# JiaweiXu8/AD-GS

Measured on AMD Instinct MI355X. Metric: fwd+bwd frames/s, higher is better.
Workload: dtype f32; 1 GPU; C3: 1000000 Gaussians, 1920x1280, SH deg 3, 8 dynamic objects, flow+semantic outputs, 1 camera/GPU/step; P=1000000, camera_pool=16 cameras / time stamps per GPU, cycled one per step (train.py:55-61), settle_steps=123, capacity_reruns=0, launch=eager, parallelism=single GPU, gradient_exchange=none, camera_streams=1

## Files before the change

ad-gs_amd/adgs/_lib.py:

```python
import contextlib
import ctypes
import os

_HERE = os.path.dirname(os.path.abspath(__file__))
PKG_ROOT = os.path.dirname(_HERE)
LIB_PATH = os.environ.get("ADGS_LIB") or os.path.join(PKG_ROOT, "lib", "libadgs_hip.so")

ALLOC_FN = ctypes.CFUNCTYPE(ctypes.c_void_p, ctypes.c_void_p, ctypes.c_size_t)

_lib = None

c_p = ctypes.c_void_p
c_i = ctypes.c_int
c_f = ctypes.c_float

SIGNATURES = {
    "adgs_last_error": (ctypes.c_char_p, []),
    "adgs_device_check": (c_i, []),
    "adgs_raster_forward": (c_i, [ALLOC_FN, c_p, ALLOC_FN, c_p, ALLOC_FN, c_p, c_i, c_i, c_i, c_i, c_p, c_i, c_i,
                                  c_p, c_p, c_p, c_p, c_p, c_p, c_p, c_f, c_p, c_p, c_p, c_p, c_p, c_f, c_f, c_i,
                                  c_p, c_p, c_p, c_p, c_p, c_i, c_p, c_i, c_p]),
    "adgs_raster_render": (c_i, [ALLOC_FN, c_p, ALLOC_FN, c_p, ALLOC_FN, c_p, c_i, c_i, c_i, c_i, c_p, c_i, c_i,
                                 c_p, c_p, c_p, c_p, c_p, c_p, c_p, c_f, c_p, c_p, c_p, c_p, c_p, c_f, c_f, c_i,
                                 c_p, c_p, c_p, c_p, c_p, c_i, c_p, c_i, c_p]),
# ... 128 lines not shown
    "adgs_mesh_normals_temp_bytes": (ctypes.c_size_t, [ctypes.c_longlong, ctypes.c_longlong]),
    "adgs_mesh_vertex_normals": (c_i, [c_i, c_i, c_p, c_p, c_p, c_p, c_p]),
    "adgs_geometry_grid_temp_bytes": (ctypes.c_size_t, [ctypes.c_longlong]),
    "adgs_geometry_grid_plan": (c_i, [c_i, c_p, c_f, c_p, c_p, c_p, c_p, c_p]),
    "adgs_geometry_grid_build": (c_i, [c_i, c_p, c_f, c_p, c_p, c_p, c_p, c_p, c_p, c_p, c_p]),
    "adgs_geometry_nearest_temp_bytes": (ctypes.c_size_t, [ctypes.c_longlong]),
    "adgs_geometry_nearest": (c_i, [c_i, c_i, c_p, c_f, c_f, c_p, c_p, c_p, c_p, c_p, c_p, c_p, c_p, c_p, c_p]),
    "adgs_geometry_face_areas": (c_i, [c_i, c_i, c_p, c_p, c_p, c_p]),
    "adgs_geometry_sample": (c_i, [c_i, c_i, c_i, c_p, c_p, c_p, ctypes.c_double, ctypes.c_ulonglong, c_p, c_p, c_p]),
    "adgs_geometry_stats_temp_bytes": (ctypes.c_size_t, [ctypes.c_longlong]),
    "adgs_geometry_distance_stats": (c_i, [c_i, c_p, c_i, c_p, ctypes.c_double, c_p, c_p, c_p]),
    "adgs_simplify_cluster_temp_bytes": (ctypes.c_size_t, [ctypes.c_longlong, ctypes.c_longlong]),
    "adgs_simplify_cluster": (c_i, [c_i, c_i, c_p, c_p, c_f, c_p, c_p, c_p, c_p, c_p]),
    "adgs_simplify_cluster_emit": (c_i, [c_i, c_i, c_p, c_p, c_p, c_p, c_p, c_p, c_p, c_p, c_p, c_p, c_p]),
    "adgs_simplify_place_temp_bytes": (ctypes.c_size_t, [ctypes.c_longlong, ctypes.c_longlong]),
    "adgs_simplify_place": (c_i, [c_i, c_i, c_i, c_i, c_p, c_p, c_p, c_p, c_p, c_p, c_f, c_p, c_i, ctypes.c_double, c_p, c_p, c_p, c_p]),
    "adgs_test_v2_published_entries": (ctypes.c_longlong, [c_p, c_i, c_i, c_p]),
    "adgs_test_v2_scanned_candidates": (ctypes.c_longlong, [c_p, c_i, c_i, c_p]),
    "adgs_test_v2_tile_counters": (ctypes.c_longlong, [c_p, c_i, c_i, c_p, c_p, ctypes.c_longlong, c_p]),
    "adgs_test_v2_blend_batches": (ctypes.c_longlong, [c_p, c_i, c_i, c_p]),
    "adgs_test_v2_cell_ranges": (ctypes.c_longlong, [c_p, c_i, c_i, c_p, ctypes.c_longlong, c_p]),
    "adgs_test_v2_published_mask": (ctypes.c_longlong, [c_p, c_i, c_p, c_p, c_p]),
    "adgs_test_v2_geom_offsets": (c_i, [c_i, c_p]),
    "adgs_test_abi_sizeof": (ctypes.c_size_t, [c_i]),
    "adgs_test_set_capacity_hints": (None, [ctypes.c_longlong, ctypes.c_longlong]),
    "adgs_test_env_reads": (ctypes.c_ulonglong, []),
    "adgs_test_scramble_slab_bounds": (c_i, [ctypes.c_uint]),
    "adgs_test_scan_temp_bytes": (ctypes.c_size_t, [ctypes.c_size_t]),
    "adgs_test_exclusive_scan_u32": (c_i, [c_p, c_p, ctypes.c_size_t, c_p, c_p]),
    "adgs_test_sort_temp_bytes": (ctypes.c_size_t, [ctypes.c_size_t]),
    "adgs_test_sort_pairs_u64": (c_i, [c_p, c_p, c_p, c_p, ctypes.c_size_t, c_i, c_p, c_p]),
    "adgs_test_sort_pairs_u32": (c_i, [c_p, c_p, c_p, c_p, ctypes.c_size_t, c_i, c_p, c_p]),
    "adgs_test_bilagrid_path": (c_i, [c_i, c_i, c_i, c_i, c_i]),
    "adgs_test_deform_plan": (c_i, [c_p, c_i, c_i, c_i, c_p, c_p, c_p, c_p, c_p, c_p, c_p, c_p, c_p, c_p]),
}


class RasterOptions(ctypes.Structure):
    _fields_ = [("struct_bytes", ctypes.c_uint64), ("antialiasing", ctypes.c_int32)]


def raster_options(antialiasing=False):
    o = RasterOptions()
    o.struct_bytes = ctypes.sizeof(RasterOptions)
    o.antialiasing = 1 if antialiasing else 0
    return o
# ... 106 lines not shown
```

ad-gs_amd/csrc/api.hip:

```cpp
#include "common.h"
#include "kernels.h"
#include "../../include/adgs_rasterizer.h"
#include "../../include/adgs_optim.h"

#include <atomic>
#include <chrono>
#include <mutex>
#include <vector>
#include <cstdlib>
#include <algorithm>
#include <cmath>
#include <cstring>

namespace adgs {

static thread_local std::string g_last_error;
struct FrameContext {
	adgs_frame_stats stats;
	size_t hint_cells, hint_fine;
	unsigned hint_max_cell_chunks;
	bool bucket_frame_pending;
	long long reruns;
	int last_order_hint;
	uint32_t* slab_bounds;
// ... 236 lines not shown
			if (captured) return nullptr;
			for (Entry& c : entries) if (!c.captured && (!e || c.used < e->used)) e = &c;
			if (!e) return nullptr;
			(void)hipStreamSynchronize(e->stream);
			if (e->tiles != tiles || e->extra != extra) { (void)hipFree(e->buf); e->buf = nullptr; e->tiles = 0; e->view = nullptr; if (hipMalloc((void**)&e->buf, (tiles + 16 + extra) * sizeof(uint32_t)) != hipSuccess) { e->buf = nullptr; return nullptr; } }
		} else {
			Entry fresh{ nullptr, nullptr, 0, 0, 0, nullptr, false, nullptr, 0, false, 0 };
			if (hipMalloc((void**)&fresh.buf, (tiles + 16 + extra) * sizeof(uint32_t)) != hipSuccess) return nullptr;
			entries.push_back(fresh);
			e = &entries.back();
		}
		e->view = view; e->proj = proj; e->W = W; e->H = H; e->tiles = tiles; e->stream = stream; e->captured = captured; e->used = ++clock; e->written = false; e->extra = extra;
		if (!reset_signature(e->buf, tiles, extra)) { e->view = nullptr; e->tiles = 0; (void)hipFree(e->buf); e->buf = nullptr; return nullptr; }
		return e;
	}
};
static OrderHints* order_hints() {
	constexpr int MAX_DEV = 64;
	static thread_local OrderHints hints[MAX_DEV];
	int dev = 0;
	if (hipGetDevice(&dev) != hipSuccess || dev < 0 || dev >= MAX_DEV) return nullptr;
	return &hints[dev];
}
struct FrameCfg { int v2; int cell_tiles; int ppl; int tile_order = 1; int sh_staging = 1; int timeline = 0; int order_ready = 0; int backwards = 0; int antialiasing = 0; int published = 0; int prefill = 0; };
static uint32_t frame_cfg_word(const FrameCfg& c) {
	return 0xAD600000u | ((uint32_t)(c.v2 & 1) << 19) | ((uint32_t)(c.tile_order & 1) << 18) | ((uint32_t)(c.sh_staging & 1) << 17) | ((uint32_t)(c.timeline & 1) << 16) |
	       ((uint32_t)(c.order_ready & 1) << 15) | ((uint32_t)(c.antialiasing & 1) << 14) | ((uint32_t)(c.published & 1) << 13) |
	       ((uint32_t)(c.prefill & 1) << 12) | ((uint32_t)(c.ppl & 0x7) << 8) | (uint32_t)(c.cell_tiles & 0xff);
}
static bool frame_cfg_from_word(uint32_t w, FrameCfg* c) {
	if ((w & 0xFFF00000u) != 0xAD600000u) return false;
	*c = FrameCfg{ (int)((w >> 19) & 1u), (int)(w & 0xffu), (int)((w >> 8) & 0x7u) };
	c->tile_order = (int)((w >> 18) & 1u); c->sh_staging = (int)((w >> 17) & 1u); c->timeline = (int)((w >> 16) & 1u); c->order_ready = (int)((w >> 15) & 1u);
	c->antialiasing = (int)((w >> 14) & 1u); c->published = (int)((w >> 13) & 1u); c->prefill = (int)((w >> 12) & 1u) & c->published;
	return c->cell_tiles >= 1 && (c->ppl == 1 || c->ppl == 2 || c->ppl == 4);
}
struct FrameKey {
	const void* img; const void* geom; int W, H, P;
	bool operator==(const FrameKey& o) const { return img == o.img && geom == o.geom && W == o.W && H == o.H && P == o.P; }
};
static std::mutex g_cfg_mu;
static std::vector<std::pair<FrameKey, FrameCfg>> g_cfg_table;
static void remember_frame(const FrameKey& k, const FrameCfg& c) {
	std::lock_guard<std::mutex> lk(g_cfg_mu);
	for (auto it = g_cfg_table.begin(); it != g_cfg_table.end();) it = (it->first.img == k.img || it->first.geom == k.geom) ? g_cfg_table.erase(it) : it + 1;
	if (g_cfg_table.size() >= 256) g_cfg_table.erase(g_cfg_table.begin());
	g_cfg_table.emplace_back(k, c);
}
static int note_backward(const FrameKey& k) {
	std::lock_guard<std::mutex> lk(g_cfg_mu);
	for (auto it = g_cfg_table.rbegin(); it != g_cfg_table.rend(); ++it) if (it->first == k) return it->second.backwards++;
	return -1;
}
static bool lookup_frame(const FrameKey& k, FrameCfg* c) {
	std::lock_guard<std::mutex> lk(g_cfg_mu);
	for (auto it = g_cfg_table.rbegin(); it != g_cfg_table.rend(); ++it) if (it->first == k) { *c = it->second; return true; }
	return false;
// ... 145 lines not shown
		size_t gb = 0, ib = 0;
		const size_t count_cells = buckets ? ncells : 0;
		const bool with_ddir = training && sh_src && M == 16;
		GeomStateV2::carve(nullptr, P, &gb, with_ddir, count_cells);
		char* gch = geometryBuffer(geometryUser, gb);
		const int ppl = v2_pixels_per_lane(ntiles), sub = TILE_Y / (4 * ppl);
		const int wgy = (height + 4 * ppl - 1) / (4 * ppl);
		const size_t wtiles = (size_t)gx * wgy;
		ImgStateV2::carve(nullptr, npix, wtiles, ncells, &ib);
		char* ich = imageBuffer(imageUser, ib);
		if (!gch || !ich) { set_error("buffer allocator returned NULL"); return -1; }
		GeomStateV2 geom = GeomStateV2::carve(gch, P, nullptr, with_ddir, count_cells);
		ImgStateV2 img = ImgStateV2::carve(ich, npix, wtiles, ncells, nullptr);
		uint32_t frame_word = 0; bool order_tiles = false;
		{
			FrameCfg fcfg{ 1, cell_tiles, ppl };
			fcfg.antialiasing = antialiasing ? 1 : 0;
			fcfg.tile_order = env_int("ADGS_TILE_ORDER", 1) != 0; fcfg.sh_staging = env_str("ADGS_NO_SH_STAGING") == nullptr; fcfg.timeline = env_int("ADGS_TIMELINE_BWD", 0) != 0;
			order_tiles = wtiles >= 2048 && fcfg.tile_order;
			if (!training) order_tiles = false;
			fcfg.order_ready = order_tiles ? 1 : 0;
			fcfg.published = (training && env_int("ADGS_PUBLISHED_MASK", 1) != 0) ? 1 : 0;
			fcfg.prefill = (fcfg.published && env_int("ADGS_GRAD_PREFILL", 1) != 0) ? 1 : 0;
			if (training) remember_frame(FrameKey{ ich, gch, width, height, P }, fcfg);
			frame_word = frame_cfg_word(fcfg);
		}
		const int fwd_order_mode = env_int("ADGS_FWD_ORDER", 2);
		OrderHints::Entry* hint = nullptr;
		const uint32_t* hint_read = nullptr;
		const bool fwd_hint_wanted = wtiles >= 2048 && env_int("ADGS_TILE_ORDER", 1) != 0 && fwd_order_mode == 2;
		if (fwd_hint_wanted) {
			hipStreamCaptureStatus cs0 = hipStreamCaptureStatusNone;
			(void)hipStreamIsCapturing(stream, &cs0);
			if (OrderHints* oh = order_hints()) {
				const bool cap0 = cs0 == hipStreamCaptureStatusActive;
				hint = oh->find(viewmatrix, projmatrix, width, height, wtiles, stream, cap0);
				if (!hint && training) {
					hipStreamCaptureMode mode = hipStreamCaptureModeRelaxed;
					if (cap0) (void)hipThreadExchangeStreamCaptureMode(&mode);
					hint = oh->create(viewmatrix, projmatrix, width, height, wtiles, stream, cap0, std::min<size_t>(ncells, (size_t)MAX_CELLS) * SLAB_ROW);
					if (cap0) (void)hipThreadExchangeStreamCaptureMode(&mode);
					(void)hipGetLastError();
				}
				oh->lookups++;
				if (hint && hint->buf) { hint_read = hint->buf; if (hint->written) oh->hits++; fc->last_order_hint = hint->written ? 1 : 0; } else { hint = nullptr; fc->last_order_hint = 0; }
			}
// ... 354 lines not shown
		ra.tile_order = nullptr;
		ra.tl_start = cfg.timeline ? img.tile_scanned : nullptr; ra.tl_end = img.tile_batches;
		PreprocessBwdArgs pa;
		pa.P = P; pa.D = D; pa.M = M;
		pa.means3D = means3D; pa.radii = radii; pa.shs = shs; pa.clamped = geom.clamped;
		pa.scales = scales; pa.rotations = rotations; pa.scale_modifier = scale_modifier;
		pa.cov3D = cov3D_precomp;
		pa.view = viewmatrix; pa.proj = projmatrix; pa.campos = campos;
		pa.focal_y = height / (2.0f * tan_fovy); pa.focal_x = width / (2.0f * tan_fovx);
		pa.tan_fovx = tan_fovx; pa.tan_fovy = tan_fovy; pa.inv_depth = inv_depth;
		pa.dL_dmean2D = nullptr; pa.dL_dconic = nullptr; pa.dL_dcolor = nullptr; pa.dL_ddepth = nullptr;
		pa.dL_dmean3D = dL_dmean3D; pa.dL_dcov3D = dL_dcov3D; pa.dL_dsh = dL_dsh; pa.dL_dscale = dL_dscale; pa.dL_drot = dL_drot;
		pa.gacc = geom.gacc; pa.splats = geom.splats; pa.W = width; pa.H = height;
		memset(&pa.sh_src, 0, sizeof(pa.sh_src)); pa.sh_dst = ShGradDst{};
		if (sh_src) { pa.sh_src = *sh_src; if (sh_dst) pa.sh_dst = *sh_dst; }
		pa.out_mean2D = dL_dmean2D; pa.out_conic = dL_dconic; pa.out_opacity = dL_dopacity; pa.out_color = dL_dcolor; pa.out_depth = dL_ddepth;
		pa.out_flow = ra.do_flow ? dL_dflow : nullptr; pa.out_sem = ra.do_sem ? dL_dsemantic : nullptr; pa.D_S = D_S;
		pa.out_mean2D_abs = dL_dmean2D_abs;
		pa.sh_staging = cfg.sh_staging;
		pa.ddir = geom.ddir;
		pa.antialias = cfg.antialiasing;
		pa.published = cfg.published ? geom.published : nullptr;
		pa.prefill = (cfg.prefill && cfg.published) ? 1 : 0;
		const FillPlan fill = preprocess_bwd_fill_plan(pa);
		{
			StageTimer t(ST_RENDER_BWD, stream);
			if (wtiles >= 2048 && cfg.tile_order) {
				if (!cfg.order_ready && launch_tile_order((int)wtiles, img.tile_consumed, img.tile_order, stream) != 0) return -1;
				ra.tile_order = img.tile_order;
			}
			if (note_backward(fkey) != 0) ADGS_HIP_CHECK(hipMemsetAsync(geom.gacc, 0, (size_t)P * GACC_STRIDE * sizeof(float), stream));
			ra.sem_src = nullptr; ra.sem_dst = nullptr; ra.sem_stride = 0;
			if (binning_buffer && launch_render_bwd_v2(ra, stream, pa.prefill ? &fill : nullptr) != 0) return -1;
			if (!binning_buffer && pa.prefill && launch_grad_prefill(fill, stream) != 0) return -1;
			if (binning_buffer && ra.do_sem && D_S > 1) {
				ADGS_HIP_CHECK(hipMemsetAsync(dL_dsemantic, 0, (size_t)P * D_S * sizeof(float), stream));
				RenderV2BwdArgs rc = ra;
				rc.do_color = rc.do_flow = rc.do_depth = rc.do_opacity = false; rc.do_sem = true; rc.absgrad = false;
				rc.dL_dpix = nullptr; rc.dL_dpix_depth = nullptr; rc.dL_dpix_flow = nullptr; rc.dL_dpix_opacity = nullptr;
				rc.bg_image = nullptr; rc.dL_dbg_image = nullptr; rc.sem_stride = D_S;
				for (int c = 1; c < D_S; c++) {
					rc.dL_dpix_sem = dL_dpix_semantic + (size_t)c * npix; rc.sem_src = semantic + c; rc.sem_dst = dL_dsemantic + c;
					if (launch_render_bwd_v2(rc, stream) != 0) return -1;
				}
			}
		}
// ... 20 lines not shown
	ra.do_depth = dL_dpix_depth != nullptr;
	ra.do_opacity = grad_img_opacity != nullptr;
	ra.dL_dmean2D = dL_dmean2D; ra.dL_dconic = dL_dconic; ra.dL_dopacity = dL_dopacity; ra.dL_dcolor = dL_dcolor;
	ra.dL_ddepth = dL_ddepth; ra.dL_dflow = dL_dflow; ra.dL_dsem = dL_dsemantic;
	if (R > 0) {
		{ StageTimer t(ST_RENDER_BWD, stream); if (launch_render_bwd(ra, stream) != 0) return -1; }
		ADGS_LAUNCH_CHECK(debug, stream);
	}

	PreprocessBwdArgs pa;
	pa.P = P; pa.D = D; pa.M = M;
	pa.means3D = means3D; pa.radii = radii; pa.shs = shs; pa.clamped = geom.clamped;
	pa.scales = scales; pa.rotations = rotations; pa.scale_modifier = scale_modifier;
	pa.cov3D = cov3D_precomp ? cov3D_precomp : geom.cov3D;
	pa.view = viewmatrix; pa.proj = projmatrix; pa.campos = campos;
	pa.focal_y = height / (2.0f * tan_fovy); pa.focal_x = width / (2.0f * tan_fovx);
	pa.tan_fovx = tan_fovx; pa.tan_fovy = tan_fovy; pa.inv_depth = inv_depth;
	pa.dL_dmean2D = dL_dmean2D; pa.dL_dconic = dL_dconic; pa.dL_dcolor = dL_dcolor; pa.dL_ddepth = dL_ddepth;
	pa.dL_dmean3D = dL_dmean3D; pa.dL_dcov3D = dL_dcov3D; pa.dL_dsh = dL_dsh; pa.dL_dscale = dL_dscale; pa.dL_drot = dL_drot;
	if (sh_src) { set_error("the raw-SH entry points need the default (v2) pipeline (not ADGS_RASTER_MODE=classic, D_S <= ADGS_V2_MAX_SEMANTIC)"); return -1; }
	memset(&pa.sh_src, 0, sizeof(pa.sh_src)); pa.sh_dst = ShGradDst{};
	pa.gacc = nullptr; pa.splats = nullptr; pa.W = width; pa.H = height; pa.out_mean2D = nullptr; pa.out_conic = nullptr; pa.out_opacity = nullptr; pa.out_color = nullptr; pa.out_depth = nullptr;
	pa.out_flow = nullptr; pa.out_sem = nullptr; pa.D_S = D_S; pa.out_mean2D_abs = nullptr;
	pa.sh_staging = cfg.sh_staging; pa.ddir = nullptr; pa.published = nullptr; pa.prefill = 0;
	pa.antialias = cfg.antialiasing;
	if (cfg.antialiasing) { pa.out_opacity = dL_dopacity; pa.splats = geom.splats; }
	{ StageTimer t(ST_PREPROCESS_BWD, stream); if (launch_preprocess_bwd(pa, stream) != 0) return -1; }
	ADGS_LAUNCH_CHECK(debug, stream);
	return 0;
}

static int read_raster_options(const adgs_raster_options* o, const char* who, int* antialiasing) {
	*antialiasing = 0;
	if (!o) return 0;
	if (o->struct_bytes < offsetof(adgs_raster_options, antialiasing) + sizeof(int32_t) || o->struct_bytes > 4096) {
		set_error(std::string(who) + ": adgs_raster_options.struct_bytes must be sizeof(adgs_raster_options) of the caller's header"); return -1;
	}
	adgs_raster_options full;
	memset(&full, 0, sizeof(full));
	memcpy(&full, o, std::min<size_t>((size_t)o->struct_bytes, sizeof(full)));
	if (full.antialiasing != 0 && full.antialiasing != 1) { set_error(std::string(who) + ": adgs_raster_options.antialiasing must be 0 or 1"); return -1; }
	*antialiasing = full.antialiasing;
	return 0;
}

extern "C" int adgs_raster_forward_opts(
	adgs_alloc_fn geometryBuffer, void* geometryUser, adgs_alloc_fn binningBuffer, void* binningUser, adgs_alloc_fn imageBuffer, void* imageUser,
// ... 296 lines not shown
}
long long sum_tile_words(const uint32_t* d_words, size_t n, hipStream_t stream) {
	std::vector<uint32_t> h(n);
	if (hipMemcpyAsync(h.data(), d_words, n * sizeof(uint32_t), hipMemcpyDeviceToHost, stream) != hipSuccess) return -1;
	if (hipStreamSynchronize(stream) != hipSuccess) return -1;
	long long total = 0;
	for (uint32_t x : h) total += x;
	return total;
}
}
extern "C" long long adgs_test_v2_published_entries(const char* img_buffer, int width, int height, void* stream_) {
	V2ImageView v;
	if (!v2_image_view(img_buffer, width, height, &v)) return -1;
	return sum_tile_words(v.img.tile_consumed, v.wtiles, (hipStream_t)stream_);
}
extern "C" long long adgs_test_v2_published_mask(const char* geom_buffer, int P, uint8_t* out_bytes, float* out_lines, void* stream_) {
	if (!geom_buffer || P <= 0) return -1;
	const GeomStateV2 g = GeomStateV2::carve(const_cast<char*>(geom_buffer), (size_t)P, nullptr, false);
	if (out_bytes && hipMemcpyAsync(out_bytes, g.published, (size_t)P, hipMemcpyDeviceToHost, (hipStream_t)stream_) != hipSuccess) return -1;
	if (out_lines && hipMemcpyAsync(out_lines, g.gacc, (size_t)P * GACC_STRIDE * sizeof(float), hipMemcpyDeviceToHost, (hipStream_t)stream_) != hipSuccess) return -1;
	if (hipStreamSynchronize((hipStream_t)stream_) != hipSuccess) return -1;
	return (long long)P;
}
extern "C" int adgs_test_v2_geom_offsets(int P, long long* out2) {
	if (P <= 0 || !out2) return -1;
	char* const base = reinterpret_cast<char*>((uintptr_t)1 << 20);
	const GeomStateV2 g = GeomStateV2::carve(base, (size_t)P, nullptr, false);
	out2[0] = (long long)(reinterpret_cast<char*>(g.published) - base); out2[1] = (long long)(reinterpret_cast<char*>(g.gacc) - base);
	return 0;
}
extern "C" long long adgs_test_v2_tile_counters(const char* img_buffer, int width, int height, uint32_t* out_consumed, uint32_t* out_scanned, long long capacity, void* stream_) {
	V2ImageView v;
	if (!v2_image_view(img_buffer, width, height, &v)) return -1;
	if ((long long)v.wtiles > capacity) return (long long)v.wtiles;
	if (out_consumed && hipMemcpyAsync(out_consumed, v.img.tile_consumed, v.wtiles * sizeof(uint32_t), hipMemcpyDeviceToHost, (hipStream_t)stream_) != hipSuccess) return -1;
	if (out_scanned && hipMemcpyAsync(out_scanned, v.img.tile_scanned, v.wtiles * sizeof(uint32_t), hipMemcpyDeviceToHost, (hipStream_t)stream_) != hipSuccess) return -1;
	if (hipStreamSynchronize((hipStream_t)stream_) != hipSuccess) return -1;
	return (long long)v.wtiles;
}
extern "C" long long adgs_test_v2_tile_words(const char* img_buffer, int width, int height, uint32_t* out_scanned, uint32_t* out_batches, long long capacity, void* stream_) {
	V2ImageView v;
	if (!v2_image_view(img_buffer, width, height, &v)) return -1;
	if ((long long)v.wtiles > capacity) return (long long)v.wtiles;
	if (out_scanned && hipMemcpyAsync(out_scanned, v.img.tile_scanned, v.wtiles * sizeof(uint32_t), hipMemcpyDeviceToHost, (hipStream_t)stream_) != hipSuccess) return -1;
	if (out_batches && hipMemcpyAsync(out_batches, v.img.tile_batches, v.wtiles * sizeof(uint32_t), hipMemcpyDeviceToHost, (hipStream_t)stream_) != hipSuccess) return -1;
	if (hipStreamSynchronize((hipStream_t)stream_) != hipSuccess) return -1;
// ... 67 lines not shown
```

ad-gs_amd/csrc/kernels.h:

```cpp
#pragma once
#include "common.h"
#include "func_eval.h"
#include "grad_prefill.h"

namespace adgs {

struct PreprocessArgs {
	int P, D, M, D_S;
	const float* means3D; const float* scales; float scale_modifier; const float* rotations;
	const float* opacities; const float* shs; const float* cov3D_precomp; const float* colors_precomp;
	const float* flow_points; const float* semantic;
	const float* view; const float* proj; const float* campos;
	int W, H, gx, gy;
	float tan_fovx, tan_fovy, focal_x, focal_y;
	int inv_depth;
	int* radii; Splat* splats; float* cov3D; uint8_t* clamped; uint32_t* tiles_touched;
	int v2;
	uint32_t* fine_touched;
	uint4* dupinfo;
	int cell_tiles, cgx, cgy;
	ShSource sh_src;
	const float* sh0;
	float* gacc;
	unsigned long long* fine_total;
// ... 40 lines not shown
};
int launch_render_bwd(const RenderBwdArgs& a, hipStream_t stream);

struct PreprocessBwdArgs {
	int P, D, M;
	const float* means3D; const int* radii; const float* shs; const uint8_t* clamped;
	const float* scales; const float* rotations; float scale_modifier;
	const float* cov3D;
	const float* view; const float* proj; const float* campos;
	float focal_x, focal_y, tan_fovx, tan_fovy;
	int inv_depth;
	const float* dL_dmean2D; const float* dL_dconic; const float* dL_dcolor; const float* dL_ddepth;
	float* dL_dmean3D; float* dL_dcov3D; float* dL_dsh; float* dL_dscale; float* dL_drot;
	float* gacc; const Splat* splats; int W, H;
	ShSource sh_src; ShGradDst sh_dst;
	float* out_mean2D; float* out_conic; float* out_opacity; float* out_color; float* out_depth; float* out_flow; float* out_sem;
	float* out_mean2D_abs;
	int D_S;
	int sh_staging;
	const float* ddir;
	int antialias;
	const uint8_t* published;
	int prefill;
};
int launch_preprocess_bwd(const PreprocessBwdArgs& a, hipStream_t stream);
FillPlan preprocess_bwd_fill_plan(const PreprocessBwdArgs& a);

constexpr int CHUNK_WORDS = 2 + WAVE;
constexpr int CHUNK_PREV = WAVE, CHUNK_COUNT = WAVE + 1;
constexpr int POOL_BLOCK = 4;
constexpr int GACC_STRIDE = 16;
constexpr int GACC_USED = 14;

constexpr int MAX_CELLS = 1024;
constexpr int SLAB_ROW = 128;
constexpr int MAX_SLAB_LG = 7;
constexpr int SLAB_TARGET = 3072;
constexpr int SLAB_TARGET_FOREIGN = 2048;
constexpr int GS_NMAX = 4096;
constexpr int MAX_CHUNKS = 16384;
constexpr size_t count_row_stride(int nblocks) { return ((size_t)nblocks + 3u) & ~(size_t)3u; }
struct Mailbox { volatile uint32_t seq; uint32_t r_cells; unsigned long long r_fine; uint32_t oversize, n_groups, overflow, overflow_count, max_cell_chunks;
	uint32_t cap_cells; unsigned long long cap_fine; };
int launch_bin_prepare(const FramePrologue& p, hipStream_t stream);
struct CellScanArgs {
	const uint32_t* cell_count;
	uint32_t* cell_start;
	uint2* cell_ranges; int ncells;
// ... 104 lines not shown
```

ad-gs_amd/csrc/preprocess_bwd.hip:

```cpp
#include "common.h"
#include "kernels.h"
#include "geom.h"
#include "func_eval.h"
#include <cstdlib>

#ifndef ADGS_PREB_STAGE_U4
#define ADGS_PREB_STAGE_U4 12
#endif
namespace adgs {
namespace {

struct M3 { float v[3][3]; };
__device__ __forceinline__ M3 m3mul(const M3& a, const M3& b) {
	M3 r;
#pragma unroll
	for (int c = 0; c < 3; c++)
#pragma unroll
		for (int rr = 0; rr < 3; rr++)
			r.v[c][rr] = a.v[0][rr] * b.v[c][0] + a.v[1][rr] * b.v[c][1] + a.v[2][rr] * b.v[c][2];
	return r;
}
__device__ __forceinline__ M3 m3t(const M3& a) {
	M3 r;
#pragma unroll
	for (int c = 0; c < 3; c++)
#pragma unroll
// ... 11 lines not shown
	const bool rs = a.sh_src.scene_xyz != nullptr && (int)i < a.sh_src.Ns;
	in.radius = gate ? 0 : a.radii[i];
	if (!pub) return in;
	const float* pos = rs ? a.sh_src.scene_xyz : a.means3D;
	in.p[0] = pos[3 * i]; in.p[1] = pos[3 * i + 1]; in.p[2] = pos[3 * i + 2];
	const float* sc = rs ? a.sh_src.scene_scaling : a.scales;
	const float* rt = rs ? a.sh_src.scene_rotation : a.rotations;
	in.s[0] = sc[3 * i]; in.s[1] = sc[3 * i + 1]; in.s[2] = sc[3 * i + 2];
	const float4 r = *reinterpret_cast<const float4*>(rt + 4 * i);
	in.q[0] = r.x; in.q[1] = r.y; in.q[2] = r.z; in.q[3] = r.w;
	in.op = rs ? a.sh_src.scene_opacity[i] : 0.f;
	const float4* ga = reinterpret_cast<const float4*>(a.gacc + i * GACC_STRIDE);
	in.u0 = ld_stream4(ga); in.u1 = ld_stream4(ga + 1); in.u2 = ld_stream4(ga + 2); in.u3 = ld_stream4(ga + 3);
	const float4* sp = reinterpret_cast<const float4*>(a.splats + i);
	in.s0 = ld_stream4(sp); in.s1 = ld_stream4(sp + 1);
	in.clamped = a.clamped[i];
	if (a.ddir) {
#pragma unroll
		for (int k = 0; k < 9; k++) in.dd[k] = ld_stream(a.ddir + (size_t)k * a.P + i);
	}
	return in;
}

template <bool STAGED, bool AA>
__global__ void __launch_bounds__(BW_THREADS) preprocess_bwd_kernel(PreprocessBwdArgs a) {
	extern __shared__ float s_sh[];
	const int tid = threadIdx.x;
	const int base = blockIdx.x * BW_THREADS;
	const int idx = base + tid;
	const bool raw = a.sh_src.scene_dc != nullptr;
	const int nvalid = min(BW_THREADS, a.P - base);
	const bool pf = STAGED && a.gacc != nullptr && a.cov3D == nullptr && a.scales != nullptr && a.rotations != nullptr;
	const bool adam_rest = STAGED && raw && (a.sh_dst.adam.scene_rest.p != nullptr || a.sh_dst.adam.obj_rest.p != nullptr);
	const bool gate = a.gacc != nullptr && a.published != nullptr;
	bool pub = true;
	if (gate) pub = idx < a.P && a.published[idx] != 0;
	bool sparse = false;
	if (gate && a.prefill) {
		const int npub = __syncthreads_count(pub);
		sparse = prefill_group_sparse(npub, nvalid);
		if (sparse && npub == 0 && !adam_rest) return;
	}
	PreBIn in;
	const bool have_ddir = STAGED && raw && pf && a.ddir != nullptr && a.D == 3;
	if (STAGED) {
		if (raw && have_ddir) {
			in = load_preb_in(a, idx, gate, pub);
		} else if (raw) {
			stage_rows<true, ADGS_PREB_STAGE_U4>(s_sh, SH_ROW_REST, SH_ROW_REST, base, nvalid, a.sh_src.Ns, a.sh_src.scene_rest, a.sh_src.obj_rest, tid, BW_THREADS,
				[&]() { if (pf) in = load_preb_in(a, idx, gate, pub); });
		} else {
			const float4* src = reinterpret_cast<const float4*>(a.shs + (size_t)base * SH_ROW_FULL);
			constexpr int NQ4 = SH_ROW_FULL / 4;
			const int total4 = nvalid * NQ4;
			float4 v[NQ4];
#pragma unroll
			for (int u = 0; u < NQ4; u++) v[u] = ld_stream4(src + min(tid + u * BW_THREADS, total4 - 1));
			if (pf) in = load_preb_in(a, idx, gate, pub);
#pragma unroll
			for (int u = 0; u < NQ4; u++) {
				const int q = tid + u * BW_THREADS;
				if (q < total4) {
					const int g = q / NQ4, c = (q - g * NQ4) * 4;
					float* d = s_sh + g * SH_ROW_FULL_LDS + c;
					d[0] = v[u].x; d[1] = v[u].y; d[2] = v[u].z; d[3] = v[u].w;
				}
			}
// ... 308 lines not shown
		for (int k = 0; k < 3; k++) { dMt.v[0][k] *= s0; dMt.v[1][k] *= s1; dMt.v[2][k] *= s2; }
#define MT(i, j) dMt.v[i][j]
		float4 dq;
		dq.x = 2 * z * (MT(0, 1) - MT(1, 0)) + 2 * y * (MT(2, 0) - MT(0, 2)) + 2 * x * (MT(1, 2) - MT(2, 1));
		dq.y = 2 * y * (MT(1, 0) + MT(0, 1)) + 2 * z * (MT(2, 0) + MT(0, 2)) + 2 * r * (MT(1, 2) - MT(2, 1)) - 4 * x * (MT(2, 2) + MT(1, 1));
		dq.z = 2 * x * (MT(1, 0) + MT(0, 1)) + 2 * r * (MT(2, 0) - MT(0, 2)) + 2 * z * (MT(1, 2) + MT(2, 1)) - 4 * y * (MT(2, 2) + MT(0, 0));
		dq.w = 2 * r * (MT(0, 1) - MT(1, 0)) + 2 * x * (MT(2, 0) + MT(0, 2)) + 2 * y * (MT(1, 2) + MT(2, 1)) - 4 * z * (MT(1, 1) + MT(0, 0));
#undef MT
		if (rs) {
			const float qg = r * dq.x + x * dq.y + y * dq.z + z * dq.w;
			st_stream4(reinterpret_cast<float4*>(a.sh_dst.scene_rotation + 4 * (size_t)idx),
				make_float4((dq.x - r * qg) * act.inv_norm, (dq.y - x * qg) * act.inv_norm, (dq.z - y * qg) * act.inv_norm, (dq.w - z * qg) * act.inv_norm));
		} else st_stream4(reinterpret_cast<float4*>(a.dL_drot + 4 * (size_t)idx), dq);
	}
	}
	if (STAGED) {
		__syncthreads();
		if (raw && adam_rest) {
			adam_rows<4>(s_sh, SH_ROW_REST, SH_ROW_REST, base, nvalid, a.sh_src.Ns, a.sh_dst.adam.scene_rest, a.sh_dst.adam.obj_rest, a.sh_dst.adam.beta1, a.sh_dst.adam.beta2, a.sh_dst.adam.eps,
				tid, BW_THREADS);
		} else if (sparse) {
			const int lane = tid & (WAVE - 1), w0 = tid - lane;
			for (uint64_t m = __builtin_amdgcn_ballot_w64(vis); m != 0ull; m &= m - 1ull) {
				const int r = w0 + __builtin_ctzll(m), gi = base + r;
				if (raw) {
					const bool is_obj = gi >= a.sh_src.Ns;
					float* const gre = is_obj ? a.sh_dst.obj_rest : a.sh_dst.scene_rest;
					if (gre && lane < SH_ROW_REST) st_stream(gre + (size_t)(is_obj ? gi - a.sh_src.Ns : gi) * SH_ROW_REST + lane, s_sh[r * SH_ROW_REST + lane]);
				} else if (lane < SH_ROW_FULL) {
					st_stream(a.dL_dsh + (size_t)gi * SH_ROW_FULL + lane, s_sh[r * SH_ROW_FULL_LDS + lane]);
				}
			}
		} else if (raw) {
			stage_rows<false>(s_sh, SH_ROW_REST, SH_ROW_REST, base, nvalid, a.sh_src.Ns, a.sh_dst.scene_rest, a.sh_dst.obj_rest, tid, BW_THREADS);
		} else {
			float4* dst = reinterpret_cast<float4*>(a.dL_dsh + (size_t)base * SH_ROW_FULL);
			for (int q = tid; q < nvalid * (SH_ROW_FULL / 4); q += BW_THREADS) {
				const int g = q / (SH_ROW_FULL / 4), c = (q - g * (SH_ROW_FULL / 4)) * 4;
				const float* s = s_sh + g * SH_ROW_FULL_LDS + c;
				st_stream4(dst + q, make_float4(s[0], s[1], s[2], s[3]));
			}
		}
	}
}

}

// ... 17 lines not shown
		fill_plan_add(fp, a.sh_dst.scene_xyz, 3, 3, 0, Nr); fill_plan_add(fp, a.sh_dst.scene_scaling, 3, 3, 0, Nr);
		fill_plan_add(fp, a.sh_dst.scene_rotation, 4, 4, 0, Nr); fill_plan_add(fp, a.sh_dst.scene_opacity, 1, 1, 0, Nr);
	}
	tail(a.dL_dmean3D, 3);
	all(a.dL_dcov3D, 6);
	if (raw) {
		fill_plan_add(fp, a.sh_dst.scene_dc, 3, 3, 0, Ns); fill_plan_add(fp, a.sh_dst.obj_dc, 3, 3, Ns, P - Ns);
		all(a.sh_dst.rgb_factor, 3);
		const bool adam_rest = a.sh_dst.adam.scene_rest.p || a.sh_dst.adam.obj_rest.p;
		const int rest = (a.M - 1) * 3;
		if (!adam_rest) { fill_plan_add(fp, a.sh_dst.scene_rest, rest, rest, 0, Ns); fill_plan_add(fp, a.sh_dst.obj_rest, rest, rest, Ns, P - Ns); }
		const bool adam_sp = a.sh_dst.adam.scene_sp.p || a.sh_dst.adam.obj_sp.p;
		if (has_lin_host(a.sh_src.f) && !adam_sp) {
			const int row = 3 * a.sh_src.f.n_params;
			fill_plan_add(fp, a.sh_dst.scene_sp, row, row, 0, Ns); fill_plan_add(fp, a.sh_dst.obj_sp, row, row, Ns, P - Ns);
		}
	} else if (a.shs) {
		all(a.dL_dsh, a.M * 3);
	}
	if (a.scales) { tail(a.dL_dscale, 3); tail(a.dL_drot, 4); }
	return fp;
}

int launch_preprocess_bwd(const PreprocessBwdArgs& a, hipStream_t stream) {
	if (a.P == 0) return 0;
	const bool raw = a.sh_src.scene_dc != nullptr;
	const bool staged = a.M == 16 && (raw || a.shs) && a.gacc != nullptr && a.sh_staging != 0;
	const unsigned grid = (unsigned)((a.P + BW_THREADS - 1) / BW_THREADS);
	const bool adam_rest = a.sh_dst.adam.scene_rest.p || a.sh_dst.adam.obj_rest.p, adam_sp = a.sh_dst.adam.scene_sp.p || a.sh_dst.adam.obj_sp.p;
	if ((adam_rest || adam_sp) && !raw) { set_error("preprocess backward: the in-backward Adam step needs the raw-SH path"); return -1; }
	if (adam_rest && !staged) {
		set_error("preprocess backward: the in-backward Adam step of the SH `rest` tensors needs 16 SH coefficients and the LDS row staging "
		          "(the frame's forward ran with ADGS_NO_SH_STAGING, or M != 16)");
		return -1;
	}
	if (a.out_mean2D_abs && !a.gacc) { set_error("preprocess backward: the absolute mean2D gradient needs the default (v2) pipeline's accumulator lines"); return -1; }
	if (a.antialias && (!a.out_opacity || (!a.gacc && !a.splats))) { set_error("preprocess backward: the anti-aliased frame's opacity gradient has no destination"); return -1; }
	if (staged) {
		const size_t lds = (size_t)BW_THREADS * (raw ? SH_ROW_REST : SH_ROW_FULL_LDS) * sizeof(float);
		if (a.antialias) hipLaunchKernelGGL((preprocess_bwd_kernel<true, true>), dim3(grid), dim3(BW_THREADS), lds, stream, a);
		else hipLaunchKernelGGL((preprocess_bwd_kernel<true, false>), dim3(grid), dim3(BW_THREADS), lds, stream, a);
	} else {
		if (a.antialias) hipLaunchKernelGGL((preprocess_bwd_kernel<false, true>), dim3(grid), dim3(BW_THREADS), 0, stream, a);
		else hipLaunchKernelGGL((preprocess_bwd_kernel<false, false>), dim3(grid), dim3(BW_THREADS), 0, stream, a);
	}
	ADGS_HIP_CHECK(hipGetLastError());
	if (raw && has_lin_host(a.sh_src.f)) {
		const int No = a.P - a.sh_src.Ns;
		if (a.prefill && a.gacc && a.published && !adam_sp)
			return launch_lin_param_grad_rows(a.sh_src.Ns, a.sh_dst.scene_dc, a.sh_dst.scene_sp, No, a.sh_dst.obj_dc, a.sh_dst.obj_sp, 3, 3, a.sh_src.f, a.published, stream);
		if (launch_lin_param_grad2(a.sh_src.Ns, a.sh_dst.scene_dc, a.sh_dst.scene_sp, No, a.sh_dst.obj_dc, a.sh_dst.obj_sp, 3, 3, a.sh_src.f, stream,
		                           &a.sh_dst.adam.scene_sp, &a.sh_dst.adam.obj_sp, a.sh_dst.adam.beta1, a.sh_dst.adam.beta2, a.sh_dst.adam.eps) != 0) return -1;
	}
	return 0;
}

}
```

include/adgs_testing.h:

```cpp
#ifndef ADGS_TESTING_H
#define ADGS_TESTING_H
#include <stddef.h>
#include <stdint.h>
#include "adgs_deform.h"
#ifdef __cplusplus
extern "C" {
#endif
size_t adgs_test_scan_temp_bytes(size_t n);
int adgs_test_exclusive_scan_u32(const uint32_t* in, uint32_t* out, size_t n, char* temp, void* stream);
size_t adgs_test_sort_temp_bytes(size_t n);
int adgs_test_sort_pairs_u64(uint64_t* keys_in, uint64_t* keys_out, uint32_t* vals_in, uint32_t* vals_out, size_t n, int end_bit, char* temp, void* stream);
int adgs_test_sort_pairs_u32(uint32_t* keys_in, uint32_t* keys_out, uint32_t* vals_in, uint32_t* vals_out, size_t n, int end_bit, char* temp, void* stream);
long long adgs_test_v2_published_entries(const char* img_buffer, int width, int height, void* stream);
long long adgs_test_v2_scanned_candidates(const char* img_buffer, int width, int height, void* stream);
long long adgs_test_v2_tile_counters(const char* img_buffer, int width, int height, uint32_t* out_consumed, uint32_t* out_scanned, long long capacity, void* stream);
long long adgs_test_v2_blend_batches(const char* img_buffer, int width, int height, void* stream);
long long adgs_test_v2_cell_ranges(const char* img_buffer, int width, int height, uint32_t* out_ranges, long long capacity, void* stream);
long long adgs_test_v2_published_mask(const char* geom_buffer, int P, uint8_t* out_bytes, float* out_lines, void* stream);
int adgs_test_v2_geom_offsets(int P, long long* out2);

size_t adgs_test_abi_sizeof(int which);

unsigned long long adgs_test_env_reads(void);

void adgs_test_set_capacity_hints(long long pairs, long long fine_pairs);

int adgs_test_scramble_slab_bounds(unsigned seed);

int adgs_test_bilagrid_path(int L, int Hg, int Wg, int H, int W);

#define ADGS_TEST_DEFORM_PLAN_FIELDS 11
int adgs_test_deform_plan(const adgs_deform_params* p, int np_xyz, int np_xyz_flow, int np_rotation, const adgs_deform_outputs* out, const float* flow_xyz,
	const float* dL_dxyz, const float* dL_drotation, const float* dL_dopacity, const float* dL_dscales, const float* dL_dflow_xyz,
	const adgs_deform_grads* grads, int32_t* fwd, int32_t* bwd);

#ifdef __cplusplus
}
#endif
#endif
```

Before: 1128 frames/s.

## Compact sparse published Gaussians into dense span blocks in preprocess backward

Adds span blocks to the staged preprocess-backward kernel. Each span block scans BWD_SPAN groups of published-mask bytes, builds an LDS list of the published indices in sparse groups, and processes them densely. The regular per-group blocks then exit early when their group is sparse. The aim is fewer partly idle wavefronts and wasted per-block work when only a few Gaussians per group are visible. In exchange it adds extra blocks, a block-level scan with syncthreads, and scattered gathers of Gaussian data. It is on by default through ADGS_BWD_COMPACT, with a test hook to read back the span-block count.

```diff
diff --git a/ad-gs_amd/adgs/_lib.py b/ad-gs_amd/adgs/_lib.py
--- a/ad-gs_amd/adgs/_lib.py
+++ b/ad-gs_amd/adgs/_lib.py
@@ -174,6 +174,7 @@
     "adgs_test_v2_cell_ranges": (ctypes.c_longlong, [c_p, c_i, c_i, c_p, ctypes.c_longlong, c_p]),
     "adgs_test_v2_published_mask": (ctypes.c_longlong, [c_p, c_i, c_p, c_p, c_p]),
     "adgs_test_v2_geom_offsets": (c_i, [c_i, c_p]),
+    "adgs_test_preprocess_bwd_span_blocks": (c_i, []),
     "adgs_test_abi_sizeof": (ctypes.c_size_t, [c_i]),
     "adgs_test_set_capacity_hints": (None, [ctypes.c_longlong, ctypes.c_longlong]),
     "adgs_test_env_reads": (ctypes.c_ulonglong, []),
diff --git a/ad-gs_amd/csrc/api.hip b/ad-gs_amd/csrc/api.hip
--- a/ad-gs_amd/csrc/api.hip
+++ b/ad-gs_amd/csrc/api.hip
@@ -282,17 +282,18 @@
 	if (hipGetDevice(&dev) != hipSuccess || dev < 0 || dev >= MAX_DEV) return nullptr;
 	return &hints[dev];
 }
-struct FrameCfg { int v2; int cell_tiles; int ppl; int tile_order = 1; int sh_staging = 1; int timeline = 0; int order_ready = 0; int backwards = 0; int antialiasing = 0; int published = 0; int prefill = 0; };
+struct FrameCfg { int v2; int cell_tiles; int ppl; int tile_order = 1; int sh_staging = 1; int timeline = 0; int order_ready = 0; int backwards = 0; int antialiasing = 0; int published = 0; int prefill = 0; int compact = 0; };
 static uint32_t frame_cfg_word(const FrameCfg& c) {
 	return 0xAD600000u | ((uint32_t)(c.v2 & 1) << 19) | ((uint32_t)(c.tile_order & 1) << 18) | ((uint32_t)(c.sh_staging & 1) << 17) | ((uint32_t)(c.timeline & 1) << 16) |
 	       ((uint32_t)(c.order_ready & 1) << 15) | ((uint32_t)(c.antialiasing & 1) << 14) | ((uint32_t)(c.published & 1) << 13) |
-	       ((uint32_t)(c.prefill & 1) << 12) | ((uint32_t)(c.ppl & 0x7) << 8) | (uint32_t)(c.cell_tiles & 0xff);
+	       ((uint32_t)(c.prefill & 1) << 12) | ((uint32_t)(c.compact & 1) << 11) | ((uint32_t)(c.ppl & 0x7) << 8) | (uint32_t)(c.cell_tiles & 0xff);
 }
 static bool frame_cfg_from_word(uint32_t w, FrameCfg* c) {
 	if ((w & 0xFFF00000u) != 0xAD600000u) return false;
 	*c = FrameCfg{ (int)((w >> 19) & 1u), (int)(w & 0xffu), (int)((w >> 8) & 0x7u) };
 	c->tile_order = (int)((w >> 18) & 1u); c->sh_staging = (int)((w >> 17) & 1u); c->timeline = (int)((w >> 16) & 1u); c->order_ready = (int)((w >> 15) & 1u);
 	c->antialiasing = (int)((w >> 14) & 1u); c->published = (int)((w >> 13) & 1u); c->prefill = (int)((w >> 12) & 1u) & c->published;
+	c->compact = (int)((w >> 11) & 1u) & c->prefill;
 	return c->cell_tiles >= 1 && (c->ppl == 1 || c->ppl == 2 || c->ppl == 4);
 }
 struct FrameKey {
@@ -484,6 +485,7 @@
 			fcfg.order_ready = order_tiles ? 1 : 0;
 			fcfg.published = (training && env_int("ADGS_PUBLISHED_MASK", 1) != 0) ? 1 : 0;
 			fcfg.prefill = (fcfg.published && env_int("ADGS_GRAD_PREFILL", 1) != 0) ? 1 : 0;
+			fcfg.compact = (fcfg.prefill && env_int("ADGS_BWD_COMPACT", 1) != 0) ? 1 : 0;
 			if (training) remember_frame(FrameKey{ ich, gch, width, height, P }, fcfg);
 			frame_word = frame_cfg_word(fcfg);
 		}
@@ -884,6 +886,7 @@
 		pa.antialias = cfg.antialiasing;
 		pa.published = cfg.published ? geom.published : nullptr;
 		pa.prefill = (cfg.prefill && cfg.published) ? 1 : 0;
+		pa.compact = (cfg.compact && pa.prefill) ? 1 : 0; pa.span_blocks = 0;
 		const FillPlan fill = preprocess_bwd_fill_plan(pa);
 		{
 			StageTimer t(ST_RENDER_BWD, stream);
@@ -950,7 +953,7 @@
 	memset(&pa.sh_src, 0, sizeof(pa.sh_src)); pa.sh_dst = ShGradDst{};
 	pa.gacc = nullptr; pa.splats = nullptr; pa.W = width; pa.H = height; pa.out_mean2D = nullptr; pa.out_conic = nullptr; pa.out_opacity = nullptr; pa.out_color = nullptr; pa.out_depth = nullptr;
 	pa.out_flow = nullptr; pa.out_sem = nullptr; pa.D_S = D_S; pa.out_mean2D_abs = nullptr;
-	pa.sh_staging = cfg.sh_staging; pa.ddir = nullptr; pa.published = nullptr; pa.prefill = 0;
+	pa.sh_staging = cfg.sh_staging; pa.ddir = nullptr; pa.published = nullptr; pa.prefill = 0; pa.compact = 0; pa.span_blocks = 0;
 	pa.antialias = cfg.antialiasing;
 	if (cfg.antialiasing) { pa.out_opacity = dL_dopacity; pa.splats = geom.splats; }
 	{ StageTimer t(ST_PREPROCESS_BWD, stream); if (launch_preprocess_bwd(pa, stream) != 0) return -1; }
@@ -1293,6 +1296,7 @@
 	if (hipStreamSynchronize((hipStream_t)stream_) != hipSuccess) return -1;
 	return (long long)P;
 }
+extern "C" int adgs_test_preprocess_bwd_span_blocks(void) { return preprocess_bwd_last_span_blocks(); }
 extern "C" int adgs_test_v2_geom_offsets(int P, long long* out2) {
 	if (P <= 0 || !out2) return -1;
 	char* const base = reinterpret_cast<char*>((uintptr_t)1 << 20);
diff --git a/ad-gs_amd/csrc/kernels.h b/ad-gs_amd/csrc/kernels.h
--- a/ad-gs_amd/csrc/kernels.h
+++ b/ad-gs_amd/csrc/kernels.h
@@ -86,8 +86,11 @@
 	int antialias;
 	const uint8_t* published;
 	int prefill;
+	int compact;
+	int span_blocks;
 };
 int launch_preprocess_bwd(const PreprocessBwdArgs& a, hipStream_t stream);
+int preprocess_bwd_last_span_blocks();
 FillPlan preprocess_bwd_fill_plan(const PreprocessBwdArgs& a);
 
 constexpr int CHUNK_WORDS = 2 + WAVE;
diff --git a/ad-gs_amd/csrc/preprocess_bwd.hip b/ad-gs_amd/csrc/preprocess_bwd.hip
--- a/ad-gs_amd/csrc/preprocess_bwd.hip
+++ b/ad-gs_amd/csrc/preprocess_bwd.hip
@@ -2,6 +2,7 @@
 #include "kernels.h"
 #include "geom.h"
 #include "func_eval.h"
+#include <atomic>
 #include <cstdlib>
 
 #ifndef ADGS_PREB_STAGE_U4
@@ -59,27 +60,91 @@
 	return in;
 }
 
+__host__ __device__ __forceinline__ bool preb_have_ddir(const PreprocessBwdArgs& a, const bool staged) {
+	return staged && a.sh_src.scene_dc != nullptr && a.gacc != nullptr && a.cov3D == nullptr && a.scales != nullptr && a.rotations != nullptr && a.ddir != nullptr && a.D == 3;
+}
+
+#ifndef ADGS_BWD_SPAN
+#define ADGS_BWD_SPAN 8
+#endif
+constexpr int BWD_SPAN = ADGS_BWD_SPAN;
+constexpr int SPAN_LIST = BWD_SPAN * (BW_THREADS / 2);
+constexpr int SPAN_PASSES = SPAN_LIST / BW_THREADS;
+static_assert(BWD_SPAN == 4 || BWD_SPAN == 8 || BWD_SPAN == 16, "a thread reads its BWD_SPAN mask bytes with one load");
+static_assert(BW_THREADS == PREFILL_GROUP, "the preprocess backward's block is the prefill's group");
+
+__device__ __forceinline__ int span_list(const uint8_t* __restrict__ published, const int P, const int sbase, const int first, const int tid, uint16_t* s_list, int* s_wave) {
+	constexpr int MB = BWD_SPAN, TPG = BW_THREADS / BWD_SPAN;
+	const int o = sbase + tid * MB;
+	uint32_t w[MB / 4];
+#pragma unroll
+	for (int i = 0; i < MB / 4; i++) w[i] = 0u;
+	if (o + MB <= P && (reinterpret_cast<uintptr_t>(published) & (uintptr_t)(MB - 1)) == 0) {
+		__builtin_memcpy(w, __builtin_assume_aligned(published + o, MB), MB);
+	} else {
+		for (int b = 0; b < MB; b++) if (o + b < P) w[b >> 2] |= (uint32_t)published[o + b] << (8 * (b & 3));
+	}
+	uint32_t m = 0u;
+#pragma unroll
+	for (int b = 0; b < MB; b++) if ((w[b >> 2] >> (8 * (b & 3))) & 0xffu) m |= 1u << b;
+	const int c = __popc(m);
+	int ng = c;
+#pragma unroll
+	for (int off = TPG / 2; off > 0; off >>= 1) ng += __shfl_xor(ng, off, WAVE);
+	const int gbase = sbase + (tid / TPG) * PREFILL_GROUP;
+	const bool sparse = prefill_group_sparse(ng, min(PREFILL_GROUP, P - gbase));
+	const int e = sparse ? c : 0;
+	const int lane = tid & (WAVE - 1), wv = tid / WAVE;
+	int incl = e;
+#pragma unroll
+	for (int off = 1; off < WAVE; off <<= 1) { const int u = __shfl_up(incl, off, WAVE); if (lane >= off) incl += u; }
+	if (lane == WAVE - 1) s_wave[wv] = incl;
+	__syncthreads();
+	int at = incl - e, n = 0;
+#pragma unroll
+	for (int i = 0; i < BW_THREADS / WAVE; i++) { if (i < wv) at += s_wave[i]; n += s_wave[i]; }
+	if (first >= n) return n;
+	if (sparse) {
+#pragma unroll
+		for (int b = 0; b < MB; b++) if ((m >> b) & 1u) s_list[at++] = (uint16_t)(tid * MB + b);
+	}
+	__syncthreads();
+	return n;
+}
+
 template <bool STAGED, bool AA>
 __global__ void __launch_bounds__(BW_THREADS) preprocess_bwd_kernel(PreprocessBwdArgs a) {
 	extern __shared__ float s_sh[];
 	const int tid = threadIdx.x;
-	const int base = blockIdx.x * BW_THREADS;
-	const int idx = base + tid;
+	const bool span = STAGED && (int)blockIdx.x < a.span_blocks;
+	const int base = span ? 0 : (STAGED ? (int)blockIdx.x - a.span_blocks : (int)blockIdx.x) * BW_THREADS;
+	int idx = base + tid;
 	const bool raw = a.sh_src.scene_dc != nullptr;
 	const int nvalid = min(BW_THREADS, a.P - base);
 	const bool pf = STAGED && a.gacc != nullptr && a.cov3D == nullptr && a.scales != nullptr && a.rotations != nullptr;
 	const bool adam_rest = STAGED && raw && (a.sh_dst.adam.scene_rest.p != nullptr || a.sh_dst.adam.obj_rest.p != nullptr);
 	const bool gate = a.gacc != nullptr && a.published != nullptr;
 	bool pub = true;
-	if (gate) pub = idx < a.P && a.published[idx] != 0;
+	if (gate && !span) pub = idx < a.P && a.published[idx] != 0;
 	bool sparse = false;
-	if (gate && a.prefill) {
+	__shared__ uint16_t s_list[STAGED ? SPAN_LIST : 1];
+	__shared__ int s_lwave[BW_THREADS / WAVE];
+	int sbase = 0, lfirst = 0;
+	if (span) {
+		const int nspans = a.span_blocks / SPAN_PASSES, pass = (int)blockIdx.x / nspans;
+		sbase = ((int)blockIdx.x - pass * nspans) * (BWD_SPAN * BW_THREADS); lfirst = pass * BW_THREADS;
+		const int nlist = span_list(a.published, a.P, sbase, lfirst, tid, s_list, s_lwave);
+		if (lfirst >= nlist) return;
+		pub = lfirst + tid < nlist;
+		idx = pub ? sbase + (int)s_list[lfirst + tid] : a.P;
+		sparse = true;
+	} else if (gate && a.prefill) {
 		const int npub = __syncthreads_count(pub);
 		sparse = prefill_group_sparse(npub, nvalid);
-		if (sparse && npub == 0 && !adam_rest) return;
+		if (sparse && (npub == 0 || (STAGED && a.span_blocks != 0)) && !adam_rest) return;
 	}
 	PreBIn in;
-	const bool have_ddir = STAGED && raw && pf && a.ddir != nullptr && a.D == 3;
+	const bool have_ddir = STAGED && raw && pf && preb_have_ddir(a, STAGED);
 	if (STAGED) {
 		if (raw && have_ddir) {
 			in = load_preb_in(a, idx, gate, pub);
@@ -434,7 +499,7 @@
 		} else if (sparse) {
 			const int lane = tid & (WAVE - 1), w0 = tid - lane;
 			for (uint64_t m = __builtin_amdgcn_ballot_w64(vis); m != 0ull; m &= m - 1ull) {
-				const int r = w0 + __builtin_ctzll(m), gi = base + r;
+				const int r = w0 + __builtin_ctzll(m), gi = span ? sbase + (int)s_list[lfirst + r] : base + r;
 				if (raw) {
 					const bool is_obj = gi >= a.sh_src.Ns;
 					float* const gre = is_obj ? a.sh_dst.obj_rest : a.sh_dst.scene_rest;
@@ -498,6 +563,9 @@
 	return fp;
 }
 
+static std::atomic<int> g_last_span_blocks{ 0 };
+int preprocess_bwd_last_span_blocks() { return g_last_span_blocks.load(std::memory_order_relaxed); }
+
 int launch_preprocess_bwd(const PreprocessBwdArgs& a, hipStream_t stream) {
 	if (a.P == 0) return 0;
 	const bool raw = a.sh_src.scene_dc != nullptr;
@@ -514,9 +582,14 @@
 	if (a.antialias && (!a.out_opacity || (!a.gacc && !a.splats))) { set_error("preprocess backward: the anti-aliased frame's opacity gradient has no destination"); return -1; }
 	if (staged) {
 		const size_t lds = (size_t)BW_THREADS * (raw ? SH_ROW_REST : SH_ROW_FULL_LDS) * sizeof(float);
-		if (a.antialias) hipLaunchKernelGGL((preprocess_bwd_kernel<true, true>), dim3(grid), dim3(BW_THREADS), lds, stream, a);
-		else hipLaunchKernelGGL((preprocess_bwd_kernel<true, false>), dim3(grid), dim3(BW_THREADS), lds, stream, a);
+		PreprocessBwdArgs k = a;
+		k.span_blocks = (a.compact && a.prefill && a.published && preb_have_ddir(a, true) && !adam_rest) ? (int)((grid + BWD_SPAN - 1) / BWD_SPAN) * SPAN_PASSES : 0;
+		const dim3 g(grid + (unsigned)k.span_blocks);
+		g_last_span_blocks.store(k.span_blocks, std::memory_order_relaxed);
+		if (a.antialias) hipLaunchKernelGGL((preprocess_bwd_kernel<true, true>), g, dim3(BW_THREADS), lds, stream, k);
+		else hipLaunchKernelGGL((preprocess_bwd_kernel<true, false>), g, dim3(BW_THREADS), lds, stream, k);
 	} else {
+		g_last_span_blocks.store(0, std::memory_order_relaxed);
 		if (a.antialias) hipLaunchKernelGGL((preprocess_bwd_kernel<false, true>), dim3(grid), dim3(BW_THREADS), 0, stream, a);
 		else hipLaunchKernelGGL((preprocess_bwd_kernel<false, false>), dim3(grid), dim3(BW_THREADS), 0, stream, a);
 	}
diff --git a/include/adgs_testing.h b/include/adgs_testing.h
--- a/include/adgs_testing.h
+++ b/include/adgs_testing.h
@@ -18,6 +18,7 @@
 long long adgs_test_v2_cell_ranges(const char* img_buffer, int width, int height, uint32_t* out_ranges, long long capacity, void* stream);
 long long adgs_test_v2_published_mask(const char* geom_buffer, int P, uint8_t* out_bytes, float* out_lines, void* stream);
 int adgs_test_v2_geom_offsets(int P, long long* out2);
+int adgs_test_preprocess_bwd_span_blocks(void);
 
 size_t adgs_test_abi_sizeof(int which);
 
```

New measurement: 1145 frames/s, median of 4. 1.02x the previous value.
